# lazytiger/pbrt-rs

Measured on AMD Instinct MI355X. Metric: Mrays/s, higher is better.
Workload: dtype f32

## Files before the change

pbrt-rs_amd/csrc/render.hip:

```cpp
#include <hip/hip_runtime.h>
#include "abi_guard.h"

#include <algorithm>
#include <chrono>
#include <cstdio>
#include <cstdlib>
#include <cstring>
#include <string>
#include <thread>
#include <vector>

#include "scene.h"
#include "trace.h"
#include "wavefront.h"

using namespace pb;

extern "C" int pbrt_hip_render_device(PbrtHipScene* s, const PbrtCamera* camera, const PbrtRenderParams* params,
                                      float* d_film, PbrtRenderStats* stats) try {
    if (!s || !camera || !params || !d_film) return PBRT_HIP_ERR_INVALID;
    PB_ENTER(s->ctx);
    HIP_TRY(s->ctx, hipSetDevice(s->ctx->device));
    return wavefront_render(s, *camera, *params, d_film, stats);
}
// ... 616 lines not shown
        origins.resize(n_mine);
        pbrt_hip_tile_partition_order(rp.x0, rp.y0, rp.x1, rp.y1, rank, world, rp.tile_order, (int32_t*)origins.data(), n_mine, &n_mine);
    }
    PbrtRenderStats local{};
    if (origins.empty()) {
        HIP_TRY(ctx, hipStreamSynchronize(st));
        if (stats) *stats = local;
        return PBRT_HIP_OK;
    }
    const int n_pix = (int)origins.size() * kTile * kTile;
    int64_t valid_pixels = 0;
    for (const int2& o : origins)
        valid_pixels += (int64_t)(std::min(o.x + kTile, rp.x1) - o.x) * (std::min(o.y + kTile, rp.y1) - o.y);
    if (li_mode) valid_pixels = li->n;
    if (export_mode) rp.spp_per_pass = rp.spp;
    int spp_pass = rp.spp_per_pass > 0 ? rp.spp_per_pass : 0;
    if (spp_pass == 0) {
        size_t free_b = 0, total_b = 0;
        HIP_TRY(ctx, hipMemGetInfo(&free_b, &total_b));
        for (const auto& b : ctx->block_cache)
            if (!b.in_use) free_b += b.bytes;
        const int64_t per_path = 400 + (rp.integrator != PBRT_INTEGRATOR_PATH ? 24 + 48ll * std::max(1, rp.max_depth) : 0);
        const int64_t target_paths = std::max<int64_t>(1ll << 20, std::min<int64_t>(1ll << 28, (int64_t)(free_b / 2) / per_path));
        spp_pass = (int)std::max<int64_t>(1, std::min<int64_t>(rp.spp, target_paths / n_pix));
    }
    spp_pass = std::min(spp_pass, rp.spp);
    if (export_mode && spp_pass != rp.spp) return invalid("camera rays: too many samples for one pass");
    const size_t N = (size_t)n_pix * spp_pass;
    if (N * 4 >= (1ull << 32)) return invalid("too many concurrent paths for 32-bit queue entries; lower spp_per_pass");

    DevBuf buf(ctx);
    bool ok = true;
    PathState ps;
    ps.n_paths = N;
    ps.two_level = s->d.bvh.instanced ? 1 : 0;
    ps.ray = buf.alloc<float4>(N * 6, &ok);
    ps.hit = buf.alloc<float4>(N * 6, &ok);
    ps.rng = buf.alloc<uint64_t>(N, &ok);
    ps.L = buf.alloc<float4>(N, &ok);
    ps.beta = buf.alloc<float4>(N, &ok);
    ps.nee_a = buf.alloc<float4>(N, &ok);
    ps.nee_f = buf.alloc<float4>(N, &ok);
    ps.nee_b = buf.alloc<float4>(N, &ok);
    ps.nee_light = buf.alloc<int>(N, &ok);
    ps.pfilm = buf.alloc<float2>(N, &ok);
    Queues q[2];
    for (int k = 0; k < 2; ++k) {
        q[k].trace = buf.alloc<uint32_t>(N * 3, &ok);
        q[k].shade = buf.alloc<uint32_t>(N, &ok);
        q[k].counts64 = buf.alloc<unsigned long long>(2, &ok);
        q[k].keys = nullptr;
        for (int a = 0; a < 3; ++a) {
            const float lo = s->d.bvh.root_min[a], hi = s->d.bvh.root_max[a];
            q[k].key_lo[a] = lo;
            q[k].key_inv[a] = hi > lo ? 1.0f / (hi - lo) : 0.0f;
        }
    }
    if (rp.ray_order < 0 || rp.ray_order > 1) return invalid("ray_order must be 0 (Morton order from the second bounce on) or 1 (queue order)");
    const bool sort_rays = rp.ray_order == 0 && rp.integrator == PBRT_INTEGRATOR_PATH;
    constexpr int sort_from = 2;
    uint32_t *sort_keys[2] = {nullptr, nullptr}, *sort_vals = nullptr;
    void* sort_tmp = nullptr;
    size_t sort_tmp_bytes = 0;
    if (sort_rays) {
// ... 20 lines not shown
        shade_sorted = buf.alloc<uint32_t>(N, &ok);
        if (pb::sort_pairs_u32(st, nullptr, &shade_tmp_bytes, shade_keys[0], shade_keys[1], shade_sorted, shade_sorted, N, 3) != 0)
            return invalid("rocPRIM radix sort: size query failed");
        shade_tmp = buf.alloc<char>(shade_tmp_bytes, &ok);
    }
    DirectState ds{};
    std::vector<int> prefix(s->d.n_lights + 1, 0);
    for (int i = 0; i < s->d.n_lights; ++i)
        prefix[i + 1] = prefix[i] + (tabulated ? round_count(s->light_samples[i]) : s->light_samples[i]);
    SamplerParams smp{};
    smp.kind = rp.sampler;
    smp.n_dims = rp.sampler_dims;
    smp.nx = rp.sampler_x;
    smp.ny = rp.sampler_y;
    smp.jitter = rp.sampler_jitter;
    ps.samp = buf.alloc<int>(N, &ok);
    if (rp.sampler == PBRT_SAMPLER_HALTON) {
        smp.n_dims = 0;
        if (!ctx->d_halton_primes) {
            std::vector<uint32_t> primes;
            std::vector<uint16_t> perms;
            halton_host_tables(&primes, &perms);
            HIP_TRY(ctx, hipMalloc((void**)&ctx->d_halton_primes, primes.size() * sizeof(uint32_t)));
            HIP_TRY(ctx, hipMalloc((void**)&ctx->d_halton_perms, perms.size() * sizeof(uint16_t)));
            HIP_TRY(ctx, hipMemcpy(ctx->d_halton_primes, primes.data(), primes.size() * sizeof(uint32_t), hipMemcpyHostToDevice));
            HIP_TRY(ctx, hipMemcpy(ctx->d_halton_perms, perms.data(), perms.size() * sizeof(uint16_t), hipMemcpyHostToDevice));
        }
        smp.primes = ctx->d_halton_primes;
        smp.perms = ctx->d_halton_perms;
        int32_t sb[4];
        pbrt_hip_sample_bounds(rp.width, rp.height, frx, fry, sb);
// ... 272 lines not shown
{
                dim3 sg((n_shade + 255) / 256), sb(256);
                if (rp.integrator == PBRT_INTEGRATOR_DIRECT && s->glossy)
                    hipLaunchKernelGGL((k_shade_direct<PBRT_INTEGRATOR_DIRECT, true>), sg, sb, 0, st, sc, ps, ds, q[cur], q[nxt], pp, tiles, n_shade);
                else if (rp.integrator == PBRT_INTEGRATOR_DIRECT)
                    hipLaunchKernelGGL((k_shade_direct<PBRT_INTEGRATOR_DIRECT, false>), sg, sb, 0, st, sc, ps, ds, q[cur], q[nxt], pp, tiles, n_shade);
                else if (rp.integrator == PBRT_INTEGRATOR_WHITTED && s->glossy)
                    hipLaunchKernelGGL((k_shade_direct<PBRT_INTEGRATOR_WHITTED, true>), sg, sb, 0, st, sc, ps, ds, q[cur], q[nxt], pp, tiles, n_shade);
                else if (rp.integrator == PBRT_INTEGRATOR_WHITTED)
                    hipLaunchKernelGGL((k_shade_direct<PBRT_INTEGRATOR_WHITTED, false>), sg, sb, 0, st, sc, ps, ds, q[cur], q[nxt], pp, tiles, n_shade);
                else
                    hipLaunchKernelGGL((k_shade_direct<PBRT_INTEGRATOR_AO, false>), sg, sb, 0, st, sc, ps, ds, q[cur], q[nxt], pp, tiles, n_shade);
            }
            else {
                Queues qin = q[cur];
                if (sort_shade && wavefront >= 1 && n_shade >= (1u << 10)) {
                    hipLaunchKernelGGL(k_shade_sort_keys, dim3((n_shade + 255) / 256), dim3(256), 0, st, sc, ps, q[cur].shade, n_shade,
                                       pp.max_depth, shade_keys[0]);
                    size_t tb = shade_tmp_bytes;
                    if (pb::sort_pairs_u32(st, shade_tmp, &tb, shade_keys[0], shade_keys[1], q[cur].shade, shade_sorted, n_shade, 3) != 0 &&
                        rc == PBRT_HIP_OK) {
                        ctx->last_error = "rocPRIM radix sort failed";
                        rc = PBRT_HIP_ERR_DEVICE;
                    }
                    qin.shade = shade_sorted;
                }
                const dim3 sg((n_shade + 255) / 256), sb(256);
                if (bin_shade && wavefront >= 1 && s->glossy)
                    hipLaunchKernelGGL((k_shade<true, true>), sg, sb, 0, st, sc, ps, qin, q[nxt], pp, tiles, n_shade);
                else if (bin_shade && wavefront >= 1)
                    hipLaunchKernelGGL((k_shade<true, false>), sg, sb, 0, st, sc, ps, qin, q[nxt], pp, tiles, n_shade);
                else if (s->glossy)
                    hipLaunchKernelGGL((k_shade<false, true>), sg, sb, 0, st, sc, ps, qin, q[nxt], pp, tiles, n_shade);
                else
                    hipLaunchKernelGGL((k_shade<false, false>), sg, sb, 0, st, sc, ps, qin, q[nxt], pp, tiles, n_shade);
            }
            RENDER_TRY(hipGetLastError());
            RENDER_TRY(hipMemcpyAsync(ctx->h_counts, q[nxt].counts64, sizeof(counts), hipMemcpyDeviceToHost, st));
            RENDER_TRY(hipEventRecord(ctx->ev_sync, st));
            if (rc == PBRT_HIP_OK) {
                hipError_t qe;
                const auto spin_start = std::chrono::steady_clock::now();
                uint32_t polls = 0;
                while ((qe = hipEventQuery(ctx->ev_sync)) == hipErrorNotReady) {
                    if ((++polls & 0xfffu) == 0) {
                        const double waited = std::chrono::duration<double>(std::chrono::steady_clock::now() - spin_start).count();
                        if (waited > ctx->wavefront_deadline_s) {
                            ctx->last_error = "a wavefront did not finish within the deadline (hung kernel?)";
                            ctx->lost = true;
                            rc = PBRT_HIP_ERR_DEVICE;
                            break;
                        }
                        if (waited > 0.05) std::this_thread::yield();
                    }
                }
                if (rc == PBRT_HIP_OK) RENDER_TRY(qe);
            }
            counts[0] = ctx->h_counts[0];
            counts[1] = ctx->h_counts[1];
            if (n_trace > 0 && rc == PBRT_HIP_OK) {
                float ms = 0.0f;
                RENDER_TRY(hipEventElapsedTime(&ms, e_t0, e_t1));
                local.trace_ms += ms;
                local.trace_launches += 1;
                if (ctx->trace_log)
                    std::fprintf(stderr, "[pbrt_hip] k_trace: %u rays %.3f ms (%.0f Mrays/s)\n", n_trace, ms, n_trace / ms * 1e-3);
                ctx->trace_ms += ms;
                ctx->trace_launches += 1;
            }
            {
                uint64_t n_rays = counts[0] & 0xffffffffull, n_shadow = counts[0] >> 32;
                local.rays_closest += n_rays - n_shadow;
                local.rays_shadow += n_shadow;
                counts[0] = n_rays;
            }
            (void)first;
            first = false;
            wavefront += 1;
            cur = nxt;
        }
        if (li_mode) {
// ... 56 lines not shown
```

pbrt-rs_amd/csrc/wf_direct.h:

```cpp
#pragma once
#include "wf_path.h"

namespace pb {

struct DirectState {
    int* stage;
    float4* ld_acc;
    float4* frames;
    int light_strategy;
    int mode;
    int ao_samples;
    int ao_cos_sample;
};

#ifndef PB_DIRECT_WAVES
#define PB_DIRECT_WAVES 2
#endif
template <int MODE, bool GLOSSY>
__global__ void __launch_bounds__(256, (GLOSSY && MODE == PBRT_INTEGRATOR_DIRECT) ? 1 : PB_DIRECT_WAVES) k_shade_direct(ShadeConsts sc, PathState ps, DirectState ds, Queues qin,
                                                        Queues qout, PassParams pp, TileList tiles, uint32_t n_in) {
    uint32_t i = blockIdx.x * blockDim.x + threadIdx.x;
    bool active = i < n_in;
    uint32_t p = active ? qin.shade[i] : 0u;
    bool emit_cont = false, emit_mis = false, emit_shadow = false, mis_bool = false;
    if (active && !(__float_as_int(ps.beta[p].w) & PF_VALID)) active = false;

    if (active) {
        float4 Lq = ps.L[p], bq = ps.beta[p];
        V3 L = V3{Lq.x, Lq.y, Lq.z};
        V3 T = V3{bq.x, bq.y, bq.z};
        int fb = __float_as_int(bq.w);
        int flags = fb & 0xff, depth = fb >> 8;
        int sg = ds.stage[p];
        int stage = sg & 0xffff, sp = sg >> 16;
        float4 accq = ds.ld_acc[p];
        V3 ld_acc = V3{accq.x, accq.y, accq.z};
        size_t rbase = ray_index(ps, p, RS_CONT), hbase = hit_index(ps, p, RS_CONT);
        constexpr int mode = MODE;
        const bool sample_all = mode == PBRT_INTEGRATOR_DIRECT && ds.light_strategy == 0;
        Samp sm = path_sampler(ps, pp, tiles, p);
        const bool tabulated = pp.smp.kind != PBRT_SAMPLER_RANDOM;
        bool fallback = (sm.arr & 0x8000) != 0;
        auto stages_at_vertex = [&]() {
            return (mode == PBRT_INTEGRATOR_AO)        ? ds.ao_samples
                   : (sc.n_lights == 0)                ? 0
                   : (mode == PBRT_INTEGRATOR_WHITTED) ? sc.n_lights
                   : !sample_all                       ? 1
                   : fallback                          ? sc.n_lights
                                                       : sc.total_light_samples;
        };
        int total = stages_at_vertex();
        bool have_vertex = !(flags & PF_ALIVE);

        if (flags & (PF_NEE_SHADOW | PF_NEE_MIS)) {
            float pick_pdf;
// ... 257 lines not shown
```

pbrt-rs_amd/csrc/wf_film.h:

```cpp
#pragma once
#include "wf_direct.h"

namespace pb {

PB_DEV V3 clamp_sample_luminance(V3 L, float max_lum) {
    float y = 0.212671f * L.x + 0.715160f * L.y + 0.072169f * L.z;
    if (y > max_lum) L = L * (max_lum / y);
    return L;
}

__global__ void k_film_accumulate(PathState ps, PassParams pp, TileList tiles, float4* accum, float* d_film) {
    uint32_t pix = blockIdx.x * blockDim.x + threadIdx.x;
    if (pix >= (uint32_t)pp.n_pix) return;
    int tile = pix >> 8, within = pix & 255;
    int2 org = tiles.origin[tile];
    int x = org.x + (within & 15), y = org.y + (within >> 4);
    if (!(x >= pp.x0 && x < pp.x1 && y >= pp.y0 && y < pp.y1)) return;
    float4 acc = accum[pix];
    auto add_sample = [&](const float4 Lq, const float2 pf) {
        V3 L = V3{Lq.x, Lq.y, Lq.z};
        float yv = 0.212671f * L.x + 0.715160f * L.y + 0.072169f * L.z;
        if (__builtin_isnan(L.x) || __builtin_isnan(L.y) || __builtin_isnan(L.z) || yv < -1e-5f || __builtin_isinf(yv))
            L = V3{0.0f, 0.0f, 0.0f};
        L = clamp_sample_luminance(L, pp.max_sample_luminance);
// ... 12 lines not shown
                    float* fp = d_film + ((size_t)yy * pp.width + xx) * 4;
                    atomicAdd(fp + 0, 0.412453f * c.x + 0.357580f * c.y + 0.180423f * c.z);
                    atomicAdd(fp + 1, 0.212671f * c.x + 0.715160f * c.y + 0.072169f * c.z);
                    atomicAdd(fp + 2, 0.019334f * c.x + 0.119193f * c.y + 0.950227f * c.z);
                    atomicAdd(fp + 3, 1.0f);
                }
            }
    };
    int s = 0;
    for (; s + 4 <= pp.n_samples; s += 4) {
        float4 Lq[4];
        float2 pf[4];
#pragma unroll
        for (int k = 0; k < 4; ++k) {
            const uint32_t p = sample_pixel_to_path(pp, s + k, pix);
            Lq[k] = ps.L[p];
            pf[k] = ps.pfilm[p];
        }
#pragma unroll
        for (int k = 0; k < 4; ++k) add_sample(Lq[k], pf[k]);
    }
    for (; s < pp.n_samples; ++s) {
        const uint32_t p = sample_pixel_to_path(pp, s, pix);
        add_sample(ps.L[p], ps.pfilm[p]);
    }
    accum[pix] = acc;
}

__global__ void k_film_accumulate_rows(PathState ps, PassParams pp, TileList tiles, float4* accum, float* d_film) {
    const uint32_t t = blockIdx.x * blockDim.x + threadIdx.x;
    const uint32_t pix = t >> 4, k = t & 15u;
    if (pix >= (uint32_t)pp.n_pix) return;
    int tile = pix >> 8, within = pix & 255;
    int2 org = tiles.origin[tile];
    int x = org.x + (within & 15), y = org.y + (within >> 4);
    if (!(x >= pp.x0 && x < pp.x1 && y >= pp.y0 && y < pp.y1)) return;
    const int row0 = (int)(threadIdx.x & 63u & ~15u);
    float4 acc = accum[pix];
    for (int s0 = 0; s0 < pp.n_samples; s0 += 16) {
        const uint32_t p = sample_pixel_to_path(pp, s0 + (int)k, pix);
        const float4 Lq = ps.L[p];
        const float2 pf = ps.pfilm[p];
        V3 L = V3{Lq.x, Lq.y, Lq.z};
        float yv = 0.212671f * L.x + 0.715160f * L.y + 0.072169f * L.z;
        if (__builtin_isnan(L.x) || __builtin_isnan(L.y) || __builtin_isnan(L.z) || yv < -1e-5f || __builtin_isinf(yv))
            L = V3{0.0f, 0.0f, 0.0f};
        L = clamp_sample_luminance(L, pp.max_sample_luminance);
        float dx = pf.x - 0.5f, dy = pf.y - 0.5f;
        int px0 = max((int)__builtin_ceilf(dx - 0.5f), 0), py0 = max((int)__builtin_ceilf(dy - 0.5f), 0);
        int px1 = min((int)__builtin_floorf(dx + 0.5f) + 1, pp.width), py1 = min((int)__builtin_floorf(dy + 0.5f) + 1, pp.height);
        float own = 0.0f;
        for (int yy = py0; yy < py1; ++yy)
            for (int xx = px0; xx < px1; ++xx) {
                if (xx == x && yy == y) {
                    own = 1.0f;
                } else {
// ... 9 lines not shown
            const float w = __shfl(own, row0 + j, 64);
            if (w != 0.0f) {
                acc.x += cx;
                acc.y += cy;
                acc.z += cz;
                acc.w += 1.0f;
            }
        }
    }
    if (k == 0) accum[pix] = acc;
}

__global__ void k_film_splat(PathState ps, PassParams pp, TileList tiles, float* d_film) {
    uint32_t p = blockIdx.x * blockDim.x + threadIdx.x;
    if (p >= (uint32_t)pp.n_pix * pp.n_samples) return;
    if (!(__float_as_int(ps.beta[p].w) & PF_VALID)) return;
    float4 Lq = ps.L[p];
    V3 L = V3{Lq.x, Lq.y, Lq.z};
    float yv = 0.212671f * L.x + 0.715160f * L.y + 0.072169f * L.z;
    if (__builtin_isnan(L.x) || __builtin_isnan(L.y) || __builtin_isnan(L.z) || yv < -1e-5f || __builtin_isinf(yv))
        L = V3{0.0f, 0.0f, 0.0f};
    L = clamp_sample_luminance(L, pp.max_sample_luminance);
    float2 pf = ps.pfilm[p];
    float dx = pf.x - 0.5f, dy = pf.y - 0.5f;
    int px0 = max((int)__builtin_ceilf(dx - pp.filter_rx), 0), py0 = max((int)__builtin_ceilf(dy - pp.filter_ry), 0);
    int px1 = min((int)__builtin_floorf(dx + pp.filter_rx) + 1, pp.width);
    int py1 = min((int)__builtin_floorf(dy + pp.filter_ry) + 1, pp.height);
    const float inv_rx = 1.0f / pp.filter_rx, inv_ry = 1.0f / pp.filter_ry;
    for (int yy = py0; yy < py1; ++yy) {
        float fy = __builtin_fabsf(((float)yy - dy) * inv_ry * 16.0f);
        int ify = min(15, (int)__builtin_floorf(fy));
        for (int xx = px0; xx < px1; ++xx) {
// ... 30 lines not shown
```

pbrt-rs_amd/csrc/wf_generate_trace.h:

```cpp
#pragma once
#include "wf_sampler.h"

namespace pb {

__global__ void k_generate(PathState ps, Queues q, PassParams pp, DevCamera cam, TileList tiles) {
    uint32_t p = blockIdx.x * blockDim.x + threadIdx.x;
    uint32_t n = (uint32_t)pp.n_pix * pp.n_samples;
    if (p >= n) return;
    int s_local, pix;
    path_to_sample_pixel(pp, p, &s_local, &pix);
    int tile = pix >> 8, within = pix & 255;
    int2 org = tiles.origin[tile];
    int x = org.x + (within & 15), y = org.y + (within >> 4);
    bool valid = x >= pp.x0 && x < pp.x1 && y >= pp.y0 && y < pp.y1;
    int flags = 0;
    if (valid) {
        int s = pp.sample0 + s_local;
        Samp sm;
        rng_set_sequence(sm.rng, sample_sequence(pp, x, y, s));
        sm.pix = pix;
        sm.s = s;
        sm.dim1 = sm.dim2 = sm.arr = 0;
        sm.h_offset = pp.smp.kind == PBRT_SAMPLER_HALTON ? halton_pixel_offset(pp.smp, x, y) : 0;
        float u0, u1, l0, l1;
// ... 51 lines not shown
            float dt = dot(vabs(dw), o_err) / l2;
            ow = ow + dw * dt;
            tmax -= dt;
        }
        store_ray(ps, p, RS_CONT, ow, dw, tmax);
        samp_store(ps, p, sm);
        ps.pfilm[p] = make_float2(pfx, pfy);
        flags = PF_VALID | PF_ALIVE;
    } else {
        ps.pfilm[p] = make_float2(0.0f, 0.0f);
    }
    ps.L[p] = make_float4(0.0f, 0.0f, 0.0f, 1.0f);
    ps.beta[p] = make_float4(1.0f, 1.0f, 1.0f, __int_as_float(flags));
    if (!valid) store_ray(ps, p, RS_CONT, V3{0.0f, 0.0f, 0.0f}, V3{0.0f, 0.0f, 1.0f}, -1.0f);
    q.trace[p] = p * 4u + RS_CONT;
    q.shade[p] = p;
}

__global__ void k_li_generate(PathState ps, Queues q, const PbrtRay* __restrict__ rays, const uint64_t* __restrict__ keys, uint32_t n,
                              uint32_t n_padded, int skip) {
    uint32_t p = blockIdx.x * blockDim.x + threadIdx.x;
    if (p >= n_padded) return;
    int flags = 0;
    if (p < n) {
        Rng rng;
        rng_set_sequence(rng, keys[p]);
        for (int k = 0; k < skip; ++k) (void)rng_u32(rng);
        ps.rng[p] = rng.state;
        ps.samp[p] = 0;
        const float4* rp = reinterpret_cast<const float4*>(rays + p);
        float4 a = rp[0], b = rp[1];
        store_ray(ps, p, RS_CONT, V3{a.x, a.y, a.z}, V3{a.w, b.x, b.y}, b.z);
        flags = PF_VALID | PF_ALIVE;
    } else {
        store_ray(ps, p, RS_CONT, V3{0.0f, 0.0f, 0.0f}, V3{0.0f, 0.0f, 1.0f}, -1.0f);
    }
    ps.pfilm[p] = make_float2(0.0f, 0.0f);
    ps.L[p] = make_float4(0.0f, 0.0f, 0.0f, 1.0f);
    ps.beta[p] = make_float4(1.0f, 1.0f, 1.0f, __int_as_float(flags));
    q.trace[p] = p * 4u + RS_CONT;
    q.shade[p] = p;
}
__global__ void k_li_output(PathState ps, uint32_t n, float* __restrict__ rgb) {
    uint32_t p = blockIdx.x * blockDim.x + threadIdx.x;
    if (p >= n) return;
    float4 L = ps.L[p];
    rgb[3 * (size_t)p] = L.x;
    rgb[3 * (size_t)p + 1] = L.y;
    rgb[3 * (size_t)p + 2] = L.z;
}
__global__ void k_camera_rays_out(PathState ps, PassParams pp, TileList tiles, PbrtRay* __restrict__ rays, uint64_t* __restrict__ keys,
                                  float* __restrict__ pfilm, int32_t* __restrict__ pixel_sample) {
    uint32_t p = blockIdx.x * blockDim.x + threadIdx.x;
    uint32_t n = (uint32_t)pp.n_pix * pp.n_samples;
    if (p >= n) return;
    int s_local, pix;
    path_to_sample_pixel(pp, p, &s_local, &pix);
    int2 org = tiles.origin[pix >> 8];
    int x = org.x + (pix & 15), y = org.y + ((pix & 255) >> 4);
    bool valid = (__float_as_int(ps.beta[p].w) & PF_VALID) != 0;
    size_t ri = ray_index(ps, p, RS_CONT);
// ... 19 lines not shown
    PB_DEV uint32_t n() const { return count; }
    PB_DEV int segments() const { return n_segments; }
    PB_DEV uint32_t token(uint32_t i) const { return queue[i]; }
    PB_DEV bool strict(uint32_t e) const { return (e & 3u) == RS_MIS_BOOL; }
    PB_DEV bool load(uint32_t e, TravRay* r, bool* any) const {
        uint32_t p = e >> 2, slot = e & 3u;
        size_t ri = ray_index(ps, p, slot == RS_MIS_BOOL ? (uint32_t)RS_MIS : slot);
        float4 a = ps.ray[ri], b = ps.ray[ri + 1];
        *r = TravRay{a.x, a.y, a.z, a.w, b.x, b.y, b.z};
        *any = slot >= RS_SHADOW;
        return !(b.z < 0.0f);
    }
    PB_DEV void store(uint32_t e, bool any, bool found, float t, float b0, float b1, float b2, int slot, int inst) const {
        uint32_t p = e >> 2, rs = e & 3u;
        if (rs == RS_MIS_BOOL) {
            ps.hit[hit_index(ps, p, RS_MIS)] = make_float4(__int_as_float(found ? 0 : -1), 0.0f, 0.0f, 0.0f);
            return;
        }
        size_t ri = hit_index(ps, p, rs);
        if (any) {
            ps.hit[ri] = make_float4(found ? 1.0f : 0.0f, 0.0f, 0.0f, 0.0f);
        } else {
            (void)t;
            ps.hit[ri] = make_float4(__int_as_float(found ? slot : -1), b0, b1, b2);
            if (TWO_LEVEL) ps.hit[ri + 1] = make_float4(__int_as_float(inst), 0.0f, 0.0f, 0.0f);
        }
    }
};

template <bool COUNT, int INST, bool SPH = false>
__global__ void __launch_bounds__(kTraceBlock, (COUNT || SPH) ? 4 : (INST ? PB_INST_WAVES : PB_TRACE_WAVES))
    k_trace(DevBVH bvh, PathState ps, const uint32_t* __restrict__ queue, uint32_t n, unsigned int* work_counter,
            unsigned long long* counters, int segments) {
    __shared__ uint2 lds_stack[kStackLds * kTraceBlock];
// ... 34 lines not shown
```

pbrt-rs_amd/csrc/wf_path.h:

```cpp
#pragma once
#include "wf_lights.h"

namespace pb {

PB_DEV uint32_t shade_key(const ShadeConsts& sc, const PathState& ps, uint32_t p, int max_depth) {
    int fb = __float_as_int(ps.beta[p].w);
    uint32_t key = 0;
    if ((fb & PF_ALIVE) && (fb >> 8) < max_depth) {
        const size_t hb = hit_index(ps, p, RS_CONT);
        int slot = __float_as_int(ps.hit[hb].x), inst = hit_instance(ps, hb);
        if (slot >= 0) {
            int mat = __float_as_int(sc.bvh.tris[3 * (size_t)slot + 2].z);
            if (sc.bvh.instanced && inst >= 0) {
                int over = __float_as_int(sc.bvh.instances[7 * (size_t)inst + 6].x);
                if (over >= 0) mat = over;
            }
            key = 1u + (uint32_t)sc.materials[mat].type;
        }
    }
    return key;
}
__global__ void k_shade_sort_keys(ShadeConsts sc, PathState ps, const uint32_t* __restrict__ shade_queue, uint32_t n, int max_depth,
                                  uint32_t* __restrict__ keys) {
    uint32_t i = blockIdx.x * blockDim.x + threadIdx.x;
    if (i >= n) return;
    keys[i] = shade_key(sc, ps, shade_queue[i], max_depth);
}

constexpr int shade_keys(bool glossy) { return glossy ? 8 : 6; }
template <int KEYS>
struct ShadeBins {
    uint32_t count[4][KEYS];
    uint32_t path[256];
};

#ifndef PB_SHADE_WAVES
#define PB_SHADE_WAVES 3
#endif
template <bool BIN, bool GLOSSY>
__global__ void __launch_bounds__(256, PB_SHADE_WAVES) k_shade(ShadeConsts sc, PathState ps, Queues qin, Queues qout, PassParams pp,
                                                 TileList tiles, uint32_t n_in) {
    constexpr int kShadeKeys = shade_keys(GLOSSY);
    uint32_t i = blockIdx.x * blockDim.x + threadIdx.x;
    bool active = i < n_in;
    uint32_t p = active ? qin.shade[i] : 0u;
    if (BIN) {
        __shared__ ShadeBins<kShadeKeys> bins;
        const int lane = threadIdx.x & 63, wave = threadIdx.x >> 6;
        const uint32_t key = active ? shade_key(sc, ps, p, pp.max_depth) : (uint32_t)(kShadeKeys - 1);
        uint32_t rank = 0;
#pragma unroll
        for (int k = 0; k < kShadeKeys; ++k) {
            const unsigned long long m = __ballot(key == (uint32_t)k);
            if (key == (uint32_t)k) rank = lane_prefix(m);
            if (lane == 0) bins.count[wave][k] = (uint32_t)__popcll(m);
        }
        __syncthreads();
        uint32_t before = 0;
        for (int k = 0; k < kShadeKeys; ++k)
            for (int w = 0; w < 4; ++w)
                before += ((uint32_t)k < key || ((uint32_t)k == key && w < wave)) ? bins.count[w][k] : 0u;
        bins.path[before + rank] = p;
        uint32_t n_active = 0;
        for (int k = 0; k < kShadeKeys - 1; ++k)
            for (int w = 0; w < 4; ++w) n_active += bins.count[w][k];
        __syncthreads();
        p = bins.path[threadIdx.x];
        active = threadIdx.x < n_active;
    }
    bool emit_cont = false, emit_mis = false, emit_shadow = false, mis_bool = false;

    uint32_t cell = 0;
    if (active) {
        float4 Lq = ps.L[p], bq = ps.beta[p];
        V3 L = V3{Lq.x, Lq.y, Lq.z};
        float eta_scale = Lq.w;
        V3 beta = V3{bq.x, bq.y, bq.z};
        int fb = __float_as_int(bq.w);
        int flags = fb & 0xff, bounces = fb >> 8;
        size_t rbase = ray_index(ps, p, RS_CONT), hbase = hit_index(ps, p, RS_CONT);

        if (flags & (PF_NEE_SHADOW | PF_NEE_MIS)) {
            float pick_pdf;
            V3 beta_v;
            V3 ld = estimate_direct_resolve(sc, ps, p, flags, &pick_pdf, &beta_v);
            ld = ld / pick_pdf;
            L = L + mulv(beta_v, ld);
            flags &= ~(PF_NEE_SHADOW | PF_NEE_MIS);
        }

        if (flags & PF_ALIVE) {
            flags &= ~PF_ALIVE;
            float4 r0 = ps.ray[rbase], r1 = ps.ray[rbase + 1];
            V3 rd = V3{r0.w, r1.x, r1.y};
            float4 h0 = ps.hit[hbase];
            int hslot = __float_as_int(h0.x);
            bool found = hslot >= 0;
            Surf sf;
            if (found) {
                sf = surface_from_hit(sc.bvh, hslot, hit_instance(ps, hbase), h0.y, h0.z, h0.w, rd);
                if (qout.keys) cell = ray_sort_cell(sf.p.x, sf.p.y, sf.p.z, qout.key_lo, qout.key_inv);
            }
            if (bounces == 0 || (flags & PF_SPECULAR_BOUNCE)) {
                if (found) {
                    L = L + mulv(beta, surface_le(sc, sf, -rd));
                } else {
                    for (int k = 0; k < sc.n_infinite; ++k) {
                        DevLight lt = sc.lights[sc.infinite_ids[k]];
                        V3 le = lt.slot >= 0 ? env_le(sc.env_maps[lt.slot], rd) : V3{lt.L[0], lt.L[1], lt.L[2]};
                        L = L + mulv(beta, le);
                    }
                }
            }
            if (found && bounces < pp.max_depth) {
                DevMaterial mat = sc.materials[sf.material];
                Samp sm = path_sampler(ps, pp, tiles, p);
                if (mat.type == PBRT_MAT_NONE) {
                    V3 o = offset_ray_origin(sf.p, sf.p_error, sf.n, rd);
                    store_ray(ps, p, RS_CONT, o, rd, kInf);
                    flags |= PF_ALIVE;
                    emit_cont = true;
                } else {
                    Frame fr = make_frame(sf);
                    V3 kd = V3{mat.kd[0], mat.kd[1], mat.kd[2]};
                    V3 kt = V3{mat.kt[0], mat.kt[1], mat.kt[2]};
                    V3 wo = -rd;
                    bool has_lobe;
                    bool nonspecular;
                    NsBsdf nsb;
                    if (GLOSSY) {
                        nsb = ns_bsdf(mat);
                        nonspecular = nsb.n > 0;
                        if (mat.type == PBRT_MAT_GLASS) has_lobe = !(is_black(kd) && is_black(kt));
                        else if (mat.type == PBRT_MAT_MIRROR) has_lobe = !is_black(kd);
// ... 2 lines not shown
                        if (mat.type == PBRT_MAT_GLASS) has_lobe = !(is_black(kd) && is_black(kt));
                        else has_lobe = !is_black(kd);
                        nonspecular = (mat.type == PBRT_MAT_MATTE) && has_lobe;
                    }

                    if (nonspecular && sc.n_lights > 0) {
                        float u_pick = samp_1d(pp, sm);
                        DevDistribution1D distrib = light_distribution_lookup(sc, sf.p);
                        int light_num = find_interval_cdf(distrib.cdf, distrib.n + 1, u_pick);
                        float pick_pdf = distrib.func_int > 0.0f ? distrib.func[light_num] / (distrib.func_int * (float)distrib.n)
                                                                 : 0.0f;
                        if (pick_pdf != 0.0f) {
                            float ul0, ul1, us0, us1;
                            samp_2d(pp, sm, &ul0, &ul1);
                            samp_2d(pp, sm, &us0, &us1);
                            int nee_flags = GLOSSY ? estimate_direct_emit(sc, ps, p, sf, fr, true, nsb, light_num, ul0, ul1, us0,
                                                                          us1, pick_pdf, beta)
                                                   : estimate_direct_emit(sc, ps, p, sf, fr, true, MatteBsdf{kd}, light_num, ul0, ul1,
                                                                          us0, us1, pick_pdf, beta);
                            flags |= nee_flags & 0xff;
                            emit_shadow = (nee_flags & PF_NEE_SHADOW) != 0;
                            emit_mis = (nee_flags & PF_NEE_MIS) != 0;
                            mis_bool = (nee_flags & NEE_MIS_BOOL) != 0;
                        }
                    }

                    float u0 = 0.0f, u1 = 0.0f;
                    samp_2d(pp, sm, &u0, &u1);
                    V3 wi = V3{0.0f, 0.0f, 0.0f}, f = V3{0.0f, 0.0f, 0.0f};
                    float pdf = 0.0f;
                    bool sampled_specular = false, sampled_transmission = false;
                    if (has_lobe) {
                        if (GLOSSY && nonspecular) {
// ... 20 lines not shown
                        beta = mulv(beta, f * (absdot(wi, fr.ns) / pdf));
                        flags = (flags & ~PF_SPECULAR_BOUNCE) | (sampled_specular ? PF_SPECULAR_BOUNCE : 0);
                        if (sampled_specular && sampled_transmission) {
                            float eta = mat.eta;
                            eta_scale *= (dot(wo, sf.n) > 0.0f) ? (eta * eta) : 1.0f / (eta * eta);
                        }
                        V3 o = offset_ray_origin(sf.p, sf.p_error, sf.n, wi);
                        bool alive = true;
                        V3 rr_beta = beta * eta_scale;
                        if (max_comp(rr_beta) < pp.rr_threshold && bounces > 3) {
                            float qq = fmaxr(0.05f, 1.0f - max_comp(rr_beta));
                            if (samp_1d(pp, sm) < qq) alive = false;
                            else beta = beta / (1.0f - qq);
                        }
                        if (alive) {
                            store_ray(ps, p, RS_CONT, o, wi, kInf);
                            flags |= PF_ALIVE;
                            emit_cont = true;
                            bounces += 1;
                        }
                    }
                }
                samp_store(ps, p, sm);
            }
        }
        ps.L[p] = make_float4(L.x, L.y, L.z, eta_scale);
        ps.beta[p] = make_float4(beta.x, beta.y, beta.z, __int_as_float((bounces << 8) | flags));
    }

    __shared__ BlockAppend sh;
    const bool again = emit_cont || emit_mis || emit_shadow;
    block_append(sh, qout, p, emit_cont, emit_mis, emit_shadow, again, cell, mis_bool);
}

}
```

pbrt-rs_amd/csrc/wf_state.h:

```cpp
#pragma once
#include <hip/hip_runtime.h>

#include "scene.h"
#include "trace.h"
#include "trace_persistent.h"
#include "trace_wide.h"
#include "trace_stackless.h"

namespace pb {

constexpr int kTile = 16;
enum PathFlags : int {
    PF_SPECULAR_BOUNCE = 1,
    PF_ALIVE = 2,
    PF_NEE_SHADOW = 4,
    PF_NEE_MIS = 8,
    PF_VALID = 16,
};
enum RaySlot : int { RS_CONT = 0, RS_MIS = 1, RS_SHADOW = 2 };
constexpr uint32_t RS_MIS_BOOL = 3;
constexpr int NEE_MIS_BOOL = 0x100;

struct PathState {
    float4* ray;
    float4* hit;
    size_t n_paths;
    uint64_t* rng;
    float4* L;
    float4* beta;
    float4* nee_a;
    float4* nee_f;
    float4* nee_b;
    int* nee_light;
    float2* pfilm;
    int* samp;
    int two_level;
};
PB_DEV int hit_instance(const PathState& ps, size_t hit_base) { return ps.two_level ? __float_as_int(ps.hit[hit_base + 1].x) : -1; }

#ifndef PB_RAY_PATH_MAJOR
#define PB_RAY_PATH_MAJOR 0
#endif
#ifndef PB_HIT_PATH_MAJOR
#define PB_HIT_PATH_MAJOR 0
#endif
PB_DEV size_t ray_index(const PathState& ps, uint32_t p, int slot) {
    return PB_RAY_PATH_MAJOR ? ((size_t)p * 3 + slot) * 2 : ((size_t)slot * ps.n_paths + p) * 2;
}
PB_DEV size_t hit_index(const PathState& ps, uint32_t p, int slot) {
    return PB_HIT_PATH_MAJOR ? ((size_t)p * 3 + slot) * 2 : ((size_t)slot * ps.n_paths + p) * 2;
}

struct SamplerParams {
    int kind;
    int n_dims;
    int nx, ny, jitter;
    int n_arrays;
    int off2;
    int n_elems;
    float* tables;
    const int2* arrays;
    int h_scale[2], h_exp[2];
    int h_stride, array_end_dim;
    unsigned int h_minv[2];
    const uint16_t* perms;
// ... 101 lines not shown
    }
    __syncthreads();
    uint32_t rbase = sh.base_rays + sh.wave_rays[wave];
    uint32_t ic = rbase + lane_prefix(mc), im = rbase + wc + lane_prefix(mm), is = rbase + wc + wm + lane_prefix(ms);
    if (cont) q.trace[ic] = p * 4u + RS_CONT;
    if (mis) q.trace[im] = p * 4u + (mis_bool ? RS_MIS_BOOL : (uint32_t)RS_MIS);
    if (shadow) q.trace[is] = p * 4u + RS_SHADOW;
    if (q.keys) {
        if (cont) q.keys[ic] = cell;
        if (mis) q.keys[im] = mis_bool ? (cell | (1u << (kSortKeyBits - 1))) : cell;
        if (shadow) q.keys[is] = cell | (1u << (kSortKeyBits - 1));
    }
    if (again) q.shade[sh.base_paths + sh.wave_paths[wave] + lane_prefix(ma)] = p;
}

PB_DEV void store_ray(const PathState& ps, uint32_t p, int slot, V3 o, V3 d, float tmax) {
    size_t i = ray_index(ps, p, slot);
    ps.ray[i] = make_float4(o.x, o.y, o.z, d.x);
    ps.ray[i + 1] = make_float4(d.y, d.z, tmax, 0.0f);
}

struct DevCamera {
    float c2w[16], r2c[16];
    float lens_radius, focal_distance, shutter_open, shutter_close;
    int kind;
};
PB_DEV V3 xform_point(const float* m, V3 p) {
    float xp = m[0] * p.x + m[1] * p.y + m[2] * p.z + m[3];
    float yp = m[4] * p.x + m[5] * p.y + m[6] * p.z + m[7];
    float zp = m[8] * p.x + m[9] * p.y + m[10] * p.z + m[11];
// ... 16 lines not shown
```

pbrt-rs_amd/csrc/wf_surface.h:

```cpp
#pragma once
#include "wf_generate_trace.h"

namespace pb {

struct Surf {
    V3 p, p_error, n, dpdu, wo;
    V3 ns, sdpdu;
    int material, light;
};

PB_DEV void tri_vertices(const DevBVH& bvh, int slot, V3* p0, V3* p1, V3* p2, int* prim, int* mat, int* light) {
    float4 a = bvh.tris[3 * (size_t)slot], b = bvh.tris[3 * (size_t)slot + 1], c = bvh.tris[3 * (size_t)slot + 2];
    *p0 = V3{a.x, a.y, a.z};
    *p1 = V3{a.w, b.x, b.y};
    *p2 = V3{b.z, b.w, c.x};
    *prim = __float_as_int(c.y);
    *mat = __float_as_int(c.z);
    *light = (__float_as_int(c.w) & kPrimLightMask) - 1;
}

PB_DEV void tri_shading_geometry(const DevBVH& bvh, int slot, V3 p0, V3 p1, V3 p2, float b0, float b1, float b2, V3* n_out,
                                 V3* ns_out, V3* dpdu_out, V3* sdpdu_out) {
    float uv0x = 0.0f, uv0y = 0.0f, uv1x = 1.0f, uv1y = 0.0f, uv2x = 1.0f, uv2y = 1.0f;
    float4 s0 = make_float4(0, 0, 0, 0), s1 = s0, s2 = s0, s3 = s0, s4 = s0;
// ... 345 lines not shown
    for (int i = 0; i < 3; ++i) {
        if (mx[i] > mn[i]) o[i] /= mx[i] - mn[i];
        int v = (int)(o[i] * (float)sc.n_voxel[i]);
        pi[i] = v < 0 ? 0 : (v > sc.n_voxel[i] - 1 ? sc.n_voxel[i] - 1 : v);
    }
    size_t voxel = ((size_t)pi[2] * sc.n_voxel[1] + pi[1]) * sc.n_voxel[0] + pi[0];
    const float* t = sc.spatial + voxel * (size_t)(2 * sc.n_lights + 2);
    DevDistribution1D d;
    d.func = t;
    d.cdf = t + sc.n_lights;
    d.func_int = t[2 * sc.n_lights + 1];
    d.n = sc.n_lights;
    return d;
}

PB_DEV Samp path_sampler(const PathState& ps, const PassParams& pp, const TileList& tiles, uint32_t p) {
    Samp sm;
    if (pp.stream_keys) {
        sm.rng.inc = (pp.stream_keys[p] << 1) | 1;
        sm.rng.state = ps.rng[p];
        sm.pix = 0;
        sm.s = 0;
        sm.dim1 = sm.dim2 = sm.arr = 0;
        sm.h_offset = 0;
        return sm;
    }
    int s_local, pix;
    path_to_sample_pixel(pp, p, &s_local, &pix);
    int2 org = tiles.origin[pix >> 8];
    int x = org.x + (pix & 15), y = org.y + ((pix & 255) >> 4);
    sm.rng.inc = (sample_sequence(pp, x, y, pp.sample0 + s_local) << 1) | 1;
    sm.rng.state = ps.rng[p];
    sm.pix = pix;
    sm.s = pp.sample0 + s_local;
    int c = ps.samp[p];
    sm.dim1 = c & 0x3ff;
    sm.dim2 = (c >> 10) & 0x3f;
    sm.arr = (c >> 16) & 0xffff;
    sm.h_offset = pp.smp.kind == PBRT_SAMPLER_HALTON ? halton_pixel_offset(pp.smp, x, y) : 0;
    return sm;
}

PB_DEV Frame make_frame(const Surf& sf) {
// ... 18 lines not shown
```

Before: 2871.

## Add optional dense path-state compaction with double-buffered generations and compact hit records

Adds a compile-time dense mode for the path integrator: the shade kernel writes surviving paths into a second, compacted PathState generation through a block-level reservation, keeps an original-index map, and writes finished radiance to a separate Lfinal buffer. Generations are swapped each bounce, so shading reads a contiguous queue instead of an indirection list. Independently of that mode, hit records drop to one float4 per slot for non-instanced BVHs, and pass sizing is recomputed from actual buffer sizes with a larger share of free memory. Film splatting now checks pixel bounds instead of reading beta flags. The dense mode costs a second copy of the per-path state and extra bookkeeping, and is disabled unless PB_DENSE_STATE is defined.

```diff
diff --git a/pbrt-rs_amd/csrc/render.hip b/pbrt-rs_amd/csrc/render.hip
--- a/pbrt-rs_amd/csrc/render.hip
+++ b/pbrt-rs_amd/csrc/render.hip
@@ -654,14 +654,28 @@
         valid_pixels += (int64_t)(std::min(o.x + kTile, rp.x1) - o.x) * (std::min(o.y + kTile, rp.y1) - o.y);
     if (li_mode) valid_pixels = li->n;
     if (export_mode) rp.spp_per_pass = rp.spp;
+    const bool dense = PB_DENSE_STATE && rp.integrator == PBRT_INTEGRATOR_PATH && !export_mode;
+    const int hit_stride = s->d.bvh.instanced ? 2 : 1;
     int spp_pass = rp.spp_per_pass > 0 ? rp.spp_per_pass : 0;
     if (spp_pass == 0) {
         size_t free_b = 0, total_b = 0;
         HIP_TRY(ctx, hipMemGetInfo(&free_b, &total_b));
         for (const auto& b : ctx->block_cache)
             if (!b.in_use) free_b += b.bytes;
-        const int64_t per_path = 400 + (rp.integrator != PBRT_INTEGRATOR_PATH ? 24 + 48ll * std::max(1, rp.max_depth) : 0);
-        const int64_t target_paths = std::max<int64_t>(1ll << 20, std::min<int64_t>(1ll << 28, (int64_t)(free_b / 2) / per_path));
+        const int64_t gens = dense ? 2 : 1;
+        const int64_t per_gen = 3 * 2 * sizeof(float4)
+                                + sizeof(uint64_t) + sizeof(int)
+                                + 5 * sizeof(float4) + sizeof(int)
+                                + (dense ? sizeof(uint32_t) : 0);
+        const int64_t per_path = gens * per_gen
+                                 + 3 * hit_stride * sizeof(float4)
+                                 + sizeof(float2) + (dense ? sizeof(float4) : 0)
+                                 + 2 * 3 * sizeof(uint32_t)
+                                 + ((!dense || rp.shade_order == 2) ? 2 : 0) * sizeof(uint32_t)
+                                 + (rp.shade_order == 2 ? 3 * sizeof(uint32_t) : 0)
+                                 + 3 * 3 * sizeof(uint32_t) + 3 * sizeof(uint32_t)
+                                 + (rp.integrator != PBRT_INTEGRATOR_PATH ? 24 + 48ll * std::max(1, rp.max_depth) : 0);
+        const int64_t target_paths = std::max<int64_t>(1ll << 20, std::min<int64_t>(1ll << 28, (int64_t)(free_b / 10 * 7) / per_path));
         spp_pass = (int)std::max<int64_t>(1, std::min<int64_t>(rp.spp, target_paths / n_pix));
     }
     spp_pass = std::min(spp_pass, rp.spp);
@@ -674,20 +688,28 @@
     PathState ps;
     ps.n_paths = N;
     ps.two_level = s->d.bvh.instanced ? 1 : 0;
-    ps.ray = buf.alloc<float4>(N * 6, &ok);
-    ps.hit = buf.alloc<float4>(N * 6, &ok);
-    ps.rng = buf.alloc<uint64_t>(N, &ok);
-    ps.L = buf.alloc<float4>(N, &ok);
-    ps.beta = buf.alloc<float4>(N, &ok);
-    ps.nee_a = buf.alloc<float4>(N, &ok);
-    ps.nee_f = buf.alloc<float4>(N, &ok);
-    ps.nee_b = buf.alloc<float4>(N, &ok);
-    ps.nee_light = buf.alloc<int>(N, &ok);
+    ps.hit = buf.alloc<float4>(N * 3 * hit_stride, &ok);
     ps.pfilm = buf.alloc<float2>(N, &ok);
+    auto alloc_generation = [&](PathState& g) {
+        g.ray = buf.alloc<float4>(N * 6, &ok);
+        g.rng = buf.alloc<uint64_t>(N, &ok);
+        g.samp = buf.alloc<int>(N, &ok);
+        g.L = buf.alloc<float4>(N, &ok);
+        g.beta = buf.alloc<float4>(N, &ok);
+        g.nee_a = buf.alloc<float4>(N, &ok);
+        g.nee_f = buf.alloc<float4>(N, &ok);
+        g.nee_b = buf.alloc<float4>(N, &ok);
+        g.nee_light = buf.alloc<int>(N, &ok);
+        g.orig = dense ? buf.alloc<uint32_t>(N, &ok) : nullptr;
+    };
+    alloc_generation(ps);
+    ps.Lfinal = dense ? buf.alloc<float4>(N, &ok) : ps.L;
+    PathState ps_next = ps;
+    if (dense) alloc_generation(ps_next);
     Queues q[2];
     for (int k = 0; k < 2; ++k) {
         q[k].trace = buf.alloc<uint32_t>(N * 3, &ok);
-        q[k].shade = buf.alloc<uint32_t>(N, &ok);
+        q[k].shade = (!dense || rp.shade_order == 2) ? buf.alloc<uint32_t>(N, &ok) : nullptr;
         q[k].counts64 = buf.alloc<unsigned long long>(2, &ok);
         q[k].keys = nullptr;
         for (int a = 0; a < 3; ++a) {
@@ -738,7 +760,6 @@
     smp.nx = rp.sampler_x;
     smp.ny = rp.sampler_y;
     smp.jitter = rp.sampler_jitter;
-    ps.samp = buf.alloc<int>(N, &ok);
     if (rp.sampler == PBRT_SAMPLER_HALTON) {
         smp.n_dims = 0;
         if (!ctx->d_halton_primes) {
@@ -1041,9 +1062,12 @@
             }
             else {
                 Queues qin = q[cur];
+                if (dense) qin.shade = nullptr;
+                PathState ps_read = ps;
+                if (wavefront == 0) ps_read.orig = nullptr;
                 if (sort_shade && wavefront >= 1 && n_shade >= (1u << 10)) {
                     hipLaunchKernelGGL(k_shade_sort_keys, dim3((n_shade + 255) / 256), dim3(256), 0, st, sc, ps, q[cur].shade, n_shade,
-                                       pp.max_depth, shade_keys[0]);
+                                       pp.max_depth, shade_keys[0], dense);
                     size_t tb = shade_tmp_bytes;
                     if (pb::sort_pairs_u32(st, shade_tmp, &tb, shade_keys[0], shade_keys[1], q[cur].shade, shade_sorted, n_shade, 3) != 0 &&
                         rc == PBRT_HIP_OK) {
@@ -1054,13 +1078,14 @@
                 }
                 const dim3 sg((n_shade + 255) / 256), sb(256);
                 if (bin_shade && wavefront >= 1 && s->glossy)
-                    hipLaunchKernelGGL((k_shade<true, true>), sg, sb, 0, st, sc, ps, qin, q[nxt], pp, tiles, n_shade);
+                    hipLaunchKernelGGL((k_shade<true, true>), sg, sb, 0, st, sc, ps_read, ps_next, qin, q[nxt], pp, tiles, n_shade);
                 else if (bin_shade && wavefront >= 1)
-                    hipLaunchKernelGGL((k_shade<true, false>), sg, sb, 0, st, sc, ps, qin, q[nxt], pp, tiles, n_shade);
+                    hipLaunchKernelGGL((k_shade<true, false>), sg, sb, 0, st, sc, ps_read, ps_next, qin, q[nxt], pp, tiles, n_shade);
                 else if (s->glossy)
-                    hipLaunchKernelGGL((k_shade<false, true>), sg, sb, 0, st, sc, ps, qin, q[nxt], pp, tiles, n_shade);
+                    hipLaunchKernelGGL((k_shade<false, true>), sg, sb, 0, st, sc, ps_read, ps_next, qin, q[nxt], pp, tiles, n_shade);
                 else
-                    hipLaunchKernelGGL((k_shade<false, false>), sg, sb, 0, st, sc, ps, qin, q[nxt], pp, tiles, n_shade);
+                    hipLaunchKernelGGL((k_shade<false, false>), sg, sb, 0, st, sc, ps_read, ps_next, qin, q[nxt], pp, tiles, n_shade);
+                if (dense) std::swap(ps, ps_next);
             }
             RENDER_TRY(hipGetLastError());
             RENDER_TRY(hipMemcpyAsync(ctx->h_counts, q[nxt].counts64, sizeof(counts), hipMemcpyDeviceToHost, st));
@@ -1091,7 +1116,8 @@
                 local.trace_ms += ms;
                 local.trace_launches += 1;
                 if (ctx->trace_log)
-                    std::fprintf(stderr, "[pbrt_hip] k_trace: %u rays %.3f ms (%.0f Mrays/s)\n", n_trace, ms, n_trace / ms * 1e-3);
+                    std::fprintf(stderr, "[pbrt_hip] k_trace: %u rays %.3f ms (%.0f Mrays/s) n_shade %u\n", n_trace, ms, n_trace / ms * 1e-3,
+                                 n_shade);
                 ctx->trace_ms += ms;
                 ctx->trace_launches += 1;
             }
diff --git a/pbrt-rs_amd/csrc/wf_direct.h b/pbrt-rs_amd/csrc/wf_direct.h
--- a/pbrt-rs_amd/csrc/wf_direct.h
+++ b/pbrt-rs_amd/csrc/wf_direct.h
@@ -38,7 +38,7 @@
         size_t rbase = ray_index(ps, p, RS_CONT), hbase = hit_index(ps, p, RS_CONT);
         constexpr int mode = MODE;
         const bool sample_all = mode == PBRT_INTEGRATOR_DIRECT && ds.light_strategy == 0;
-        Samp sm = path_sampler(ps, pp, tiles, p);
+        Samp sm = path_sampler(ps, pp, tiles, p, p);
         const bool tabulated = pp.smp.kind != PBRT_SAMPLER_RANDOM;
         bool fallback = (sm.arr & 0x8000) != 0;
         auto stages_at_vertex = [&]() {
diff --git a/pbrt-rs_amd/csrc/wf_film.h b/pbrt-rs_amd/csrc/wf_film.h
--- a/pbrt-rs_amd/csrc/wf_film.h
+++ b/pbrt-rs_amd/csrc/wf_film.h
@@ -50,7 +50,7 @@
 #pragma unroll
         for (int k = 0; k < 4; ++k) {
             const uint32_t p = sample_pixel_to_path(pp, s + k, pix);
-            Lq[k] = ps.L[p];
+            Lq[k] = ps.Lfinal[p];
             pf[k] = ps.pfilm[p];
         }
 #pragma unroll
@@ -58,7 +58,7 @@
     }
     for (; s < pp.n_samples; ++s) {
         const uint32_t p = sample_pixel_to_path(pp, s, pix);
-        add_sample(ps.L[p], ps.pfilm[p]);
+        add_sample(ps.Lfinal[p], ps.pfilm[p]);
     }
     accum[pix] = acc;
 }
@@ -75,7 +75,7 @@
     float4 acc = accum[pix];
     for (int s0 = 0; s0 < pp.n_samples; s0 += 16) {
         const uint32_t p = sample_pixel_to_path(pp, s0 + (int)k, pix);
-        const float4 Lq = ps.L[p];
+        const float4 Lq = ps.Lfinal[p];
         const float2 pf = ps.pfilm[p];
         V3 L = V3{Lq.x, Lq.y, Lq.z};
         float yv = 0.212671f * L.x + 0.715160f * L.y + 0.072169f * L.z;
@@ -115,8 +115,14 @@
 __global__ void k_film_splat(PathState ps, PassParams pp, TileList tiles, float* d_film) {
     uint32_t p = blockIdx.x * blockDim.x + threadIdx.x;
     if (p >= (uint32_t)pp.n_pix * pp.n_samples) return;
-    if (!(__float_as_int(ps.beta[p].w) & PF_VALID)) return;
-    float4 Lq = ps.L[p];
+    {
+        int s_local, pix;
+        path_to_sample_pixel(pp, p, &s_local, &pix);
+        int2 org = tiles.origin[pix >> 8];
+        int x = org.x + (pix & 15), y = org.y + ((pix & 255) >> 4);
+        if (!(x >= pp.x0 && x < pp.x1 && y >= pp.y0 && y < pp.y1)) return;
+    }
+    float4 Lq = ps.Lfinal[p];
     V3 L = V3{Lq.x, Lq.y, Lq.z};
     float yv = 0.212671f * L.x + 0.715160f * L.y + 0.072169f * L.z;
     if (__builtin_isnan(L.x) || __builtin_isnan(L.y) || __builtin_isnan(L.z) || yv < -1e-5f || __builtin_isinf(yv))
diff --git a/pbrt-rs_amd/csrc/wf_generate_trace.h b/pbrt-rs_amd/csrc/wf_generate_trace.h
--- a/pbrt-rs_amd/csrc/wf_generate_trace.h
+++ b/pbrt-rs_amd/csrc/wf_generate_trace.h
@@ -89,7 +89,7 @@
     ps.beta[p] = make_float4(1.0f, 1.0f, 1.0f, __int_as_float(flags));
     if (!valid) store_ray(ps, p, RS_CONT, V3{0.0f, 0.0f, 0.0f}, V3{0.0f, 0.0f, 1.0f}, -1.0f);
     q.trace[p] = p * 4u + RS_CONT;
-    q.shade[p] = p;
+    if (q.shade) q.shade[p] = p;
 }
 
 __global__ void k_li_generate(PathState ps, Queues q, const PbrtRay* __restrict__ rays, const uint64_t* __restrict__ keys, uint32_t n,
@@ -114,12 +114,12 @@
     ps.L[p] = make_float4(0.0f, 0.0f, 0.0f, 1.0f);
     ps.beta[p] = make_float4(1.0f, 1.0f, 1.0f, __int_as_float(flags));
     q.trace[p] = p * 4u + RS_CONT;
-    q.shade[p] = p;
+    if (q.shade) q.shade[p] = p;
 }
 __global__ void k_li_output(PathState ps, uint32_t n, float* __restrict__ rgb) {
     uint32_t p = blockIdx.x * blockDim.x + threadIdx.x;
     if (p >= n) return;
-    float4 L = ps.L[p];
+    float4 L = ps.Lfinal[p];
     rgb[3 * (size_t)p] = L.x;
     rgb[3 * (size_t)p + 1] = L.y;
     rgb[3 * (size_t)p + 2] = L.z;
@@ -169,10 +169,10 @@
     PB_DEV void store(uint32_t e, bool any, bool found, float t, float b0, float b1, float b2, int slot, int inst) const {
         uint32_t p = e >> 2, rs = e & 3u;
         if (rs == RS_MIS_BOOL) {
-            ps.hit[hit_index(ps, p, RS_MIS)] = make_float4(__int_as_float(found ? 0 : -1), 0.0f, 0.0f, 0.0f);
+            ps.hit[hit_index_of<TWO_LEVEL>(ps, p, RS_MIS)] = make_float4(__int_as_float(found ? 0 : -1), 0.0f, 0.0f, 0.0f);
             return;
         }
-        size_t ri = hit_index(ps, p, rs);
+        size_t ri = hit_index_of<TWO_LEVEL>(ps, p, rs);
         if (any) {
             ps.hit[ri] = make_float4(found ? 1.0f : 0.0f, 0.0f, 0.0f, 0.0f);
         } else {
diff --git a/pbrt-rs_amd/csrc/wf_path.h b/pbrt-rs_amd/csrc/wf_path.h
--- a/pbrt-rs_amd/csrc/wf_path.h
+++ b/pbrt-rs_amd/csrc/wf_path.h
@@ -20,11 +20,12 @@
     }
     return key;
 }
-__global__ void k_shade_sort_keys(ShadeConsts sc, PathState ps, const uint32_t* __restrict__ shade_queue, uint32_t n, int max_depth,
-                                  uint32_t* __restrict__ keys) {
+__global__ void k_shade_sort_keys(ShadeConsts sc, PathState ps, uint32_t* __restrict__ shade_queue, uint32_t n, int max_depth,
+                                  uint32_t* __restrict__ keys, bool identity) {
     uint32_t i = blockIdx.x * blockDim.x + threadIdx.x;
     if (i >= n) return;
-    keys[i] = shade_key(sc, ps, shade_queue[i], max_depth);
+    if (identity) shade_queue[i] = i;
+    keys[i] = shade_key(sc, ps, identity ? i : shade_queue[i], max_depth);
 }
 
 constexpr int shade_keys(bool glossy) { return glossy ? 8 : 6; }
@@ -38,12 +39,12 @@
 #define PB_SHADE_WAVES 3
 #endif
 template <bool BIN, bool GLOSSY>
-__global__ void __launch_bounds__(256, PB_SHADE_WAVES) k_shade(ShadeConsts sc, PathState ps, Queues qin, Queues qout, PassParams pp,
-                                                 TileList tiles, uint32_t n_in) {
+__global__ void __launch_bounds__(256, PB_SHADE_WAVES) k_shade(ShadeConsts sc, PathState ps, PathState pw, Queues qin, Queues qout,
+                                                 PassParams pp, TileList tiles, uint32_t n_in) {
     constexpr int kShadeKeys = shade_keys(GLOSSY);
     uint32_t i = blockIdx.x * blockDim.x + threadIdx.x;
     bool active = i < n_in;
-    uint32_t p = active ? qin.shade[i] : 0u;
+    uint32_t p = !active ? 0u : (PB_DENSE_STATE && !qin.shade) ? i : qin.shade[i];
     if (BIN) {
         __shared__ ShadeBins<kShadeKeys> bins;
         const int lane = threadIdx.x & 63, wave = threadIdx.x >> 6;
@@ -71,14 +72,27 @@
     bool emit_cont = false, emit_mis = false, emit_shadow = false, mis_bool = false;
 
     uint32_t cell = 0;
+    float4 bq = make_float4(0.0f, 0.0f, 0.0f, 0.0f), h0 = make_float4(__int_as_float(-1), 0.0f, 0.0f, 0.0f);
+    const size_t hbase = hit_index(ps, p, RS_CONT);
+    if (active) bq = ps.beta[p];
+    if (PB_DENSE_STATE && (__float_as_int(bq.w) & PF_HOLE)) active = false;
+    if (active && (__float_as_int(bq.w) & PF_ALIVE)) h0 = ps.hit[hbase];
+    uint32_t j = p, p0 = p;
+    bool reserved = false;
+    if (PB_DENSE_STATE) {
+        __shared__ BlockReserve shr;
+        reserved = active && (__float_as_int(bq.w) & PF_ALIVE) && __float_as_int(h0.x) >= 0 && (__float_as_int(bq.w) >> 8) < pp.max_depth;
+        j = block_reserve(shr, qout, reserved);
+        if (active && ps.orig) p0 = ps.orig[p];
+    }
     if (active) {
-        float4 Lq = ps.L[p], bq = ps.beta[p];
+        float4 Lq = ps.L[p];
         V3 L = V3{Lq.x, Lq.y, Lq.z};
         float eta_scale = Lq.w;
         V3 beta = V3{bq.x, bq.y, bq.z};
         int fb = __float_as_int(bq.w);
         int flags = fb & 0xff, bounces = fb >> 8;
-        size_t rbase = ray_index(ps, p, RS_CONT), hbase = hit_index(ps, p, RS_CONT);
+        size_t rbase = ray_index(ps, p, RS_CONT);
 
         if (flags & (PF_NEE_SHADOW | PF_NEE_MIS)) {
             float pick_pdf;
@@ -93,7 +107,6 @@
             flags &= ~PF_ALIVE;
             float4 r0 = ps.ray[rbase], r1 = ps.ray[rbase + 1];
             V3 rd = V3{r0.w, r1.x, r1.y};
-            float4 h0 = ps.hit[hbase];
             int hslot = __float_as_int(h0.x);
             bool found = hslot >= 0;
             Surf sf;
@@ -114,10 +127,10 @@
             }
             if (found && bounces < pp.max_depth) {
                 DevMaterial mat = sc.materials[sf.material];
-                Samp sm = path_sampler(ps, pp, tiles, p);
+                Samp sm = path_sampler(ps, pp, tiles, p, p0);
                 if (mat.type == PBRT_MAT_NONE) {
                     V3 o = offset_ray_origin(sf.p, sf.p_error, sf.n, rd);
-                    store_ray(ps, p, RS_CONT, o, rd, kInf);
+                    store_ray(pw, j, RS_CONT, o, rd, kInf);
                     flags |= PF_ALIVE;
                     emit_cont = true;
                 } else {
@@ -150,9 +163,9 @@
                             float ul0, ul1, us0, us1;
                             samp_2d(pp, sm, &ul0, &ul1);
                             samp_2d(pp, sm, &us0, &us1);
-                            int nee_flags = GLOSSY ? estimate_direct_emit(sc, ps, p, sf, fr, true, nsb, light_num, ul0, ul1, us0,
+                            int nee_flags = GLOSSY ? estimate_direct_emit(sc, pw, j, sf, fr, true, nsb, light_num, ul0, ul1, us0,
                                                                           us1, pick_pdf, beta)
-                                                   : estimate_direct_emit(sc, ps, p, sf, fr, true, MatteBsdf{kd}, light_num, ul0, ul1,
+                                                   : estimate_direct_emit(sc, pw, j, sf, fr, true, MatteBsdf{kd}, light_num, ul0, ul1,
                                                                           us0, us1, pick_pdf, beta);
                             flags |= nee_flags & 0xff;
                             emit_shadow = (nee_flags & PF_NEE_SHADOW) != 0;
@@ -203,23 +216,32 @@
                             else beta = beta / (1.0f - qq);
                         }
                         if (alive) {
-                            store_ray(ps, p, RS_CONT, o, wi, kInf);
+                            store_ray(pw, j, RS_CONT, o, wi, kInf);
                             flags |= PF_ALIVE;
                             emit_cont = true;
                             bounces += 1;
                         }
                     }
                 }
-                samp_store(ps, p, sm);
-            }
-        }
-        ps.L[p] = make_float4(L.x, L.y, L.z, eta_scale);
-        ps.beta[p] = make_float4(beta.x, beta.y, beta.z, __int_as_float((bounces << 8) | flags));
+                samp_store(pw, j, sm);
+            }
+        }
+        if (!PB_DENSE_STATE) {
+            ps.L[p] = make_float4(L.x, L.y, L.z, eta_scale);
+            ps.beta[p] = make_float4(beta.x, beta.y, beta.z, __int_as_float((bounces << 8) | flags));
+        } else if (emit_cont || emit_mis || emit_shadow) {
+            pw.L[j] = make_float4(L.x, L.y, L.z, eta_scale);
+            pw.beta[j] = make_float4(beta.x, beta.y, beta.z, __int_as_float((bounces << 8) | flags));
+            pw.orig[j] = p0;
+        } else {
+            ps.Lfinal[p0] = make_float4(L.x, L.y, L.z, eta_scale);
+            if (reserved) pw.beta[j] = make_float4(0.0f, 0.0f, 0.0f, __int_as_float(PF_HOLE));
+        }
     }
 
     __shared__ BlockAppend sh;
     const bool again = emit_cont || emit_mis || emit_shadow;
-    block_append(sh, qout, p, emit_cont, emit_mis, emit_shadow, again, cell, mis_bool);
-}
-
-}
+    block_append(sh, qout, j, emit_cont, emit_mis, emit_shadow, PB_DENSE_STATE ? false : again, cell, mis_bool);
+}
+
+}
diff --git a/pbrt-rs_amd/csrc/wf_state.h b/pbrt-rs_amd/csrc/wf_state.h
--- a/pbrt-rs_amd/csrc/wf_state.h
+++ b/pbrt-rs_amd/csrc/wf_state.h
@@ -16,6 +16,7 @@
     PF_NEE_SHADOW = 4,
     PF_NEE_MIS = 8,
     PF_VALID = 16,
+    PF_HOLE = 32,
 };
 enum RaySlot : int { RS_CONT = 0, RS_MIS = 1, RS_SHADOW = 2 };
 constexpr uint32_t RS_MIS_BOOL = 3;
@@ -35,8 +36,14 @@
     float2* pfilm;
     int* samp;
     int two_level;
+    uint32_t* orig;
+    float4* Lfinal;
 };
 PB_DEV int hit_instance(const PathState& ps, size_t hit_base) { return ps.two_level ? __float_as_int(ps.hit[hit_base + 1].x) : -1; }
+
+#ifndef PB_DENSE_STATE
+#define PB_DENSE_STATE 0
+#endif
 
 #ifndef PB_RAY_PATH_MAJOR
 #define PB_RAY_PATH_MAJOR 0
@@ -47,8 +54,12 @@
 PB_DEV size_t ray_index(const PathState& ps, uint32_t p, int slot) {
     return PB_RAY_PATH_MAJOR ? ((size_t)p * 3 + slot) * 2 : ((size_t)slot * ps.n_paths + p) * 2;
 }
+template <bool TWO_LEVEL>
+PB_DEV size_t hit_index_of(const PathState& ps, uint32_t p, int slot) {
+    return (PB_HIT_PATH_MAJOR ? (size_t)p * 3 + slot : (size_t)slot * ps.n_paths + p) * (TWO_LEVEL ? 2 : 1);
+}
 PB_DEV size_t hit_index(const PathState& ps, uint32_t p, int slot) {
-    return PB_HIT_PATH_MAJOR ? ((size_t)p * 3 + slot) * 2 : ((size_t)slot * ps.n_paths + p) * 2;
+    return ps.two_level ? hit_index_of<true>(ps, p, slot) : hit_index_of<false>(ps, p, slot);
 }
 
 struct SamplerParams {
@@ -180,6 +191,28 @@
     if (again) q.shade[sh.base_paths + sh.wave_paths[wave] + lane_prefix(ma)] = p;
 }
 
+struct BlockReserve {
+    uint32_t wave_paths[16];
+    uint32_t base;
+};
+PB_DEV uint32_t block_reserve(BlockReserve& sh, const Queues& q, bool want) {
+    const int lane = threadIdx.x & 63, wave = threadIdx.x >> 6, n_waves = (blockDim.x + 63) >> 6;
+    const unsigned long long m = __ballot(want);
+    if (lane == 0) sh.wave_paths[wave] = (uint32_t)__popcll(m);
+    __syncthreads();
+    if (threadIdx.x == 0) {
+        uint32_t tp = 0;
+        for (int w = 0; w < n_waves; ++w) {
+            uint32_t pth = sh.wave_paths[w];
+            sh.wave_paths[w] = tp;
+            tp += pth;
+        }
+        sh.base = tp ? (uint32_t)atomicAdd(&q.counts64[1], (unsigned long long)tp) : 0u;
+    }
+    __syncthreads();
+    return sh.base + sh.wave_paths[wave] + lane_prefix(m);
+}
+
 PB_DEV void store_ray(const PathState& ps, uint32_t p, int slot, V3 o, V3 d, float tmax) {
     size_t i = ray_index(ps, p, slot);
     ps.ray[i] = make_float4(o.x, o.y, o.z, d.x);
diff --git a/pbrt-rs_amd/csrc/wf_surface.h b/pbrt-rs_amd/csrc/wf_surface.h
--- a/pbrt-rs_amd/csrc/wf_surface.h
+++ b/pbrt-rs_amd/csrc/wf_surface.h
@@ -383,10 +383,10 @@
     return d;
 }
 
-PB_DEV Samp path_sampler(const PathState& ps, const PassParams& pp, const TileList& tiles, uint32_t p) {
+PB_DEV Samp path_sampler(const PathState& ps, const PassParams& pp, const TileList& tiles, uint32_t p, uint32_t p0) {
     Samp sm;
     if (pp.stream_keys) {
-        sm.rng.inc = (pp.stream_keys[p] << 1) | 1;
+        sm.rng.inc = (pp.stream_keys[p0] << 1) | 1;
         sm.rng.state = ps.rng[p];
         sm.pix = 0;
         sm.s = 0;
@@ -395,7 +395,7 @@
         return sm;
     }
     int s_local, pix;
-    path_to_sample_pixel(pp, p, &s_local, &pix);
+    path_to_sample_pixel(pp, p0, &s_local, &pix);
     int2 org = tiles.origin[pix >> 8];
     int x = org.x + (pix & 15), y = org.y + ((pix & 255) >> 4);
     sm.rng.inc = (sample_sequence(pp, x, y, pp.sample0 + s_local) << 1) | 1;
```

Result: no change. 2873 (median of 2 runs) (+0.1%).
